# fwrnke/pseudo-3D-interpolation

Measured on AMD Instinct MI355X. Metric: POCS iterations/s on the 1024x1024x512 cube, higher is better.
Workload: dtype complex64 (f32 arithmetic)

## Files before the change

### pseudo-3d-interpolation_amd/csrc/p3d_api.hip

```cpp
#include <hip/hip_runtime.h>

#include <climits>
#include <cmath>
#include <algorithm>
#include <cstdlib>
#include <cstring>
#include <string>
#include <thread>
#include <vector>

#include "p3d.h"
#include "p3d_generic.hpp"
#include "p3d_host.hpp"
#include "p3d_internal.hpp"
#include "p3d_flex.hpp"
#include "p3d_mix_entry.hpp"
#include "p3d_resident.hpp"
#include "p3d_select.hpp"
#include "p3d_kernels.hpp"

namespace p3d {
#define P3D_DECL(n) const LineOps* get_line_ops_##n();
P3D_DECL(2) P3D_DECL(4) P3D_DECL(8) P3D_DECL(16) P3D_DECL(32) P3D_DECL(64) P3D_DECL(128) P3D_DECL(256)
P3D_DECL(512) P3D_DECL(1024) P3D_DECL(2048) P3D_DECL(4096)
// ... 226 lines not shown
{
    const int wpl = tpl >= 64 ? tpl / 64 : 1, rpw = tpl >= 64 ? 1 : 64 / tpl;
    const int unit = blockIdx.x * blockDim.x + threadIdx.x;
    if (unit >= n1 / rpw) return;
    unsigned run = rowbase[unit * rpw];
    for (int j = 0; j < 16 * wpl; ++j) {
        const size_t w = (size_t)unit * wpl * 16 + j;
        cbase[w] = run;
        run += (unsigned)__popcll(bits64[w]);
    }
}

static __global__ void pack_mask32_kernel(const uint16_t* bits, unsigned long long* bits32, int n1)
{
    const int i = blockIdx.x * blockDim.x + threadIdx.x;
    if (i >= (n1 / 2) * 32) return;
    const int k = i & 31, u = i >> 5;
    unsigned long long w = 0;
    for (int l = 0; l < 64; ++l) {
        const int row = 2 * u + (l >> 5), c = (l & 31) + 32 * k;
        w |= (unsigned long long)((bits[(size_t)row * 64 + (c & 63)] >> (c >> 6)) & 1u) << l;
    }
    bits32[i] = w;
}

static thread_local std::string g_err;

namespace p3d { void set_last_error(const char* msg) { g_err = msg; } }

struct p3d_plan {
    int device = 0;
    int nil = 0, nxl = 0, max_slices = 0;
    hipStream_t stream = nullptr;
    p3d_plan* pct_plan = nullptr;
    unsigned* pct_sel = nullptr;
    unsigned* pct_hist = nullptr;
    float* pct_frac = nullptr;
    bool generic = false;
    GenPlan gcol{}, grow{};
    static constexpr int GEN_STAT_BLOCKS = 64;
    const LineOps* ops_col = nullptr;
    const LineOps* ops_row = nullptr;
    c32 *tw_col = nullptr, *tw_row = nullptr;
    c32* work = nullptr;
    uint8_t* nzflag = nullptr;
    uint16_t* nzm = nullptr;
    unsigned long long* nzcount = nullptr;
    bool sparse_ok = false;
    double last_nonzero_fraction = -1.0;
    uint16_t* bits = nullptr;
    unsigned long long* bits64 = nullptr;
    unsigned long long* nzl = nullptr;
    unsigned* cbase = nullptr;
    unsigned long long* mbits = nullptr;
    unsigned* mbase = nullptr;
    const p3d::mix::Entry* mix_row = nullptr;
    bool mix_binary = false;
    bool use32 = false;
    unsigned long long* bits32 = nullptr;
    c32* tw32 = nullptr;
    int* flag = nullptr;
    unsigned* rowbase = nullptr;
    char* xc = nullptr;
    size_t xc_cap = 0;
    double* sums = nullptr;
    size_t sums_cap = 0;
    double* rowsum = nullptr;
    c32* tau = nullptr;
    size_t tau_cap = 0;
    int* done = nullptr;
    float* partials = nullptr;
    int tiles = 0;
    int cus = 0;
    int pipe_wgs = 0;
    int host_sw = 0;
    int flex_over = 0;
    bool no_colpipe = false;
    void* st_x = nullptr;
    void* st_out = nullptr;
    float* st_mask = nullptr;
    size_t st_cap = 0;
    struct Primed { bool valid = false; const void* x = nullptr; const float* mask = nullptr; int dtype = 0, nslices = 0, nonbinary = 0, violation = 0; unsigned nobs = 0;
                    bool real = false;
    } primed;
    double* sum0 = nullptr;
    int sorted_slices = 0;
    hipEvent_t ev0 = nullptr, ev1 = nullptr;
    std::vector<hipEvent_t> prof_events;
    double prof_col_ms = 0, prof_row_ms = 0;
    int prof_col_n = 0, prof_row_n = 0;

    size_t slice_elems() const { return (size_t)nil * nxl; }
};

static int upload_table(p3d_plan* p, const LineOps* ops, bool for_rows, int n, c32** dst)
{
    std::vector<c32> host;
    if (is_flex(ops)) {
        flex_build_table(n, host);
    } else {
        host.resize(for_rows ? (size_t)ops->row_tw_slots : (size_t)ops->col_tw_slots);
        if (for_rows) ops->build_row_tw(host.data());
        else ops->build_col_tw(host.data());
    }
    P3D_TRY(hipMalloc((void**)dst, sizeof(c32) * host.size()));
    P3D_TRY(hipMemcpy(*dst, host.data(), sizeof(c32) * host.size(), hipMemcpyHostToDevice));
    return P3D_OK;
}

extern "C" {

int p3d_abi_version(void) { return P3D_ABI_VERSION; }

const char* p3d_last_error(void) { return g_err.c_str(); }

int p3d_runtime_info(int* compiled_hip_version, int* runtime_hip_version)
{
    if (!compiled_hip_version || !runtime_hip_version) return fail(P3D_ERR_INVALID, "NULL argument");
    *compiled_hip_version = HIP_VERSION;
    P3D_TRY(hipRuntimeGetVersion(runtime_hip_version));
    return P3D_OK;
}

int p3d_device_count(int* n)
{
    if (!n) return fail(P3D_ERR_INVALID, "n is NULL");
    *n = 0;
    P3D_TRY(hipGetDeviceCount(n));
    return P3D_OK;
}

static bool generic_ok(int n) { return n >= 1 && n <= GEN_MAX_N && gen_make_plan(n).nf >= 0; }

int p3d_shape_supported(int nil, int nxl)
{
    if (find_ops(nil) != nullptr && find_ops(nxl) != nullptr) return 1;
    return (generic_ok(nil) && generic_ok(nxl)) ? 1 : 0;
}

int p3d_plan_destroy(p3d_plan* p)
{
    if (!p) return P3D_OK;
    if (p->pct_plan) p3d_plan_destroy(p->pct_plan);
    hipSetDevice(p->device);
    if (p->stream) hipStreamSynchronize(p->stream);
    void* bufs[] = {p->mbits, p->mbase, p->cbase, p->bits64, p->bits32, p->tw32, p->nzl, p->nzflag, p->nzm, p->nzcount, p->tw_col, p->tw_row, p->work, p->bits, p->flag, p->rowbase, p->xc, p->sums, p->rowsum, p->sum0, p->tau, p->pct_sel, p->pct_hist, p->pct_frac,
                    p->done,   p->partials, p->st_x, p->st_out, p->st_mask};
    for (void* b : bufs)
        if (b) hipFree(b);
    for (hipEvent_t e : p->prof_events) hipEventDestroy(e);
    if (p->ev0) hipEventDestroy(p->ev0);
    if (p->ev1) hipEventDestroy(p->ev1);
    if (p->stream) hipStreamDestroy(p->stream);
    delete p;
    return P3D_OK;
}

static int create_plan(p3d_plan** out, int device, int nil, int nxl, int max_slices, bool force_generic)
{
    if (!out) return fail(P3D_ERR_INVALID, "out is NULL");
    *out = nullptr;
    if (nil < 1 || nxl < 1 || max_slices < 1) return fail(P3D_ERR_INVALID, "nil, nxl and max_slices must be positive");
    if (max_slices > 65535) return fail(P3D_ERR_INVALID, "max_slices > 65535: split the cube into batches");
    const LineOps* oc = find_ops(nil);
    const LineOps* orow = find_ops(nxl);
    const bool generic = !oc || !orow || force_generic;
// ... 142 lines not shown
    if (!dst || !src) return fail(P3D_ERR_INVALID, "NULL argument");
    P3D_TRY(hipSetDevice(device));
    P3D_TRY(hipMemcpy(dst, src, bytes, kind == 0 ? hipMemcpyHostToDevice : kind == 1 ? hipMemcpyDeviceToHost : hipMemcpyDeviceToDevice));
    if (kind == 2) P3D_TRY(hipDeviceSynchronize());
    return P3D_OK;
}

int p3d_dev_memset(int device, void* dptr, int value, size_t bytes)
{
    if (!bytes) return P3D_OK;
    if (!dptr) return fail(P3D_ERR_INVALID, "NULL argument");
    P3D_TRY(hipSetDevice(device));
    P3D_TRY(hipMemset(dptr, value, bytes));
    P3D_TRY(hipDeviceSynchronize());
    return P3D_OK;
}

int p3d_dev_synchronize(int device)
{
    P3D_TRY(hipSetDevice(device));
    P3D_TRY(hipDeviceSynchronize());
    return P3D_OK;
}

int p3d_dev_mem_info(int device, size_t* free_bytes, size_t* total_bytes)
{
    if (!free_bytes || !total_bytes) return fail(P3D_ERR_INVALID, "NULL argument");
    if (int rc = use_device(device)) return rc;
    P3D_TRY(hipMemGetInfo(free_bytes, total_bytes));
    return P3D_OK;
}

int p3d_host_alloc(void** hptr, size_t bytes)
{
    if (!hptr) return fail(P3D_ERR_INVALID, "NULL argument");
    P3D_TRY(hipHostMalloc(hptr, bytes, hipHostMallocDefault));
    return P3D_OK;
}

int p3d_host_free(void* hptr)
{
    P3D_TRY(hipHostFree(hptr));
    return P3D_OK;
}

int p3d_memcpy_h2d(p3d_plan* p, void* dst, const void* src, size_t bytes)
{
    if (!p) return fail(P3D_ERR_INVALID, "NULL plan");
    P3D_TRY(hipSetDevice(p->device));
    P3D_TRY(hipMemcpyAsync(dst, src, bytes, hipMemcpyHostToDevice, p->stream));
    P3D_TRY(hipStreamSynchronize(p->stream));
    return P3D_OK;
}

int p3d_memcpy_d2h(p3d_plan* p, void* dst, const void* src, size_t bytes)
{
    if (!p) return fail(P3D_ERR_INVALID, "NULL plan");
    P3D_TRY(hipSetDevice(p->device));
    P3D_TRY(hipMemcpyAsync(dst, src, bytes, hipMemcpyDeviceToHost, p->stream));
    P3D_TRY(hipStreamSynchronize(p->stream));
    return P3D_OK;
}

int p3d_host_register(void* hptr, size_t bytes)
{
    if (!hptr || bytes == 0) return fail(P3D_ERR_INVALID, "NULL argument");
    const hipError_t e = hipHostRegister(hptr, bytes, hipHostRegisterDefault);
    if (e != hipSuccess) {
        (void)hipGetLastError();
        return fail(P3D_ERR_UNSUPPORTED, "hipHostRegister refused %zu bytes at %p: %s", bytes, hptr, hipGetErrorString(e));
    }
    return P3D_OK;
}

int p3d_host_unregister(void* hptr)
{
    if (!hptr) return fail(P3D_ERR_INVALID, "NULL argument");
    P3D_TRY(hipHostUnregister(hptr));
    return P3D_OK;
}

}

struct RunSwitches { bool no_pct_fused; bool no_mask_bits, no_compact, no_real, no_sparse, real_2048, no_resident, no_tstore, force_colpipe, no_colpipe; };
static RunSwitches read_switches()
{
    RunSwitches s;
    s.no_pct_fused = getenv("P3D_NO_PCT_FUSED") != nullptr;
    s.no_mask_bits = getenv("P3D_NO_MASK_BITS") != nullptr;
    s.no_compact = getenv("P3D_NO_COMPACT") != nullptr;
    s.no_real = getenv("P3D_NO_REAL") != nullptr;
    s.no_sparse = getenv("P3D_NO_SPARSE") != nullptr;
    s.real_2048 = getenv("P3D_NO_REAL_2048") == nullptr;
    s.no_resident = getenv("P3D_NO_RESIDENT") != nullptr;
    s.no_tstore = getenv("P3D_NO_TSTORE") != nullptr;
    s.force_colpipe = getenv("P3D_FORCE_COLPIPE") != nullptr;
    s.no_colpipe = getenv("P3D_NO_COLPIPE") != nullptr;
    return s;
}

static int check_batch(p3d_plan* p, int nslices)
{
    if (!p) return fail(P3D_ERR_INVALID, "NULL plan");
    p->primed.valid = false;
    p->sorted_slices = 0;
    if (nslices < 1 || nslices > p->max_slices)
        return fail(P3D_ERR_INVALID, "nslices = %d outside 1..max_slices (%d)", nslices, p->max_slices);
    return P3D_OK;
}

static RowArgs row_args(p3d_plan* p, int nslices)
{
    RowArgs r{};
    r.tw = p->tw_row;
    r.tw32 = p->tw32;
    r.n1 = p->nil;
    r.nslices = nslices;
    r.alpha = 1.0f;
    r.scale = (float)(1.0 / ((double)p->nil * (double)p->nxl));
    r.len = p->nxl;
    r.host_sw = p->host_sw;
    return r;
}

static ColArgs col_args(p3d_plan* p, int nslices)
{
    ColArgs c{};
    c.tw = p->tw_col;
    c.n2 = p->nxl;
    c.nslices = nslices;
    c.len = p->nil;
    c.cus = p->cus;
    c.host_sw = p->host_sw;
    c.flex_over = p->flex_over;
    return c;
}

static int ensure_staging(p3d_plan* p, size_t bytes_per_cube)
{
    if (p->st_cap >= bytes_per_cube && p->st_x) return P3D_OK;
    if (p->st_x) hipFree(p->st_x);
    if (p->st_out) hipFree(p->st_out);
    p->st_x = p->st_out = nullptr;
    p->st_cap = 0;
    P3D_TRY(hipMalloc(&p->st_x, bytes_per_cube));
    P3D_TRY(hipMalloc(&p->st_out, bytes_per_cube));
    if (!p->st_mask) P3D_TRY(hipMalloc((void**)&p->st_mask, sizeof(float) * p->slice_elems()));
    p->st_cap = bytes_per_cube;
    return P3D_OK;
}


static int gen_fft2(p3d_plan* p, const c32* in, c32* out, int nslices, int inverse, const int* done)
{
    const float scale = (float)(1.0 / ((double)p->nil * (double)p->nxl));
    if (!inverse) {
        P3D_TRY(gen_launch_line_fft(in, out, p->tw_row, p->grow, FWD, 1.0f, nslices, p->nil, p->nxl, true, done, p->stream));
        P3D_TRY(gen_launch_line_fft(out, out, p->tw_col, p->gcol, FWD, 1.0f, nslices, p->nil, p->nxl, false, done, p->stream));
    } else {
        P3D_TRY(gen_launch_line_fft(in, out, p->tw_col, p->gcol, INV, 1.0f, nslices, p->nil, p->nxl, false, done, p->stream));
        P3D_TRY(gen_launch_line_fft(out, out, p->tw_row, p->grow, INV, scale, nslices, p->nil, p->nxl, true, done, p->stream));
    }
    return P3D_OK;
}

static int reduce_partials(p3d_plan* p, int nslices, double* stats, int tiles = 0)
{
    if (tiles <= 0) tiles = p->tiles;
    std::vector<float> part((size_t)STATS_PARTIAL * tiles * nslices);
    P3D_TRY(hipMemcpyAsync(part.data(), p->partials, sizeof(float) * part.size(), hipMemcpyDeviceToHost, p->stream));
    P3D_TRY(hipStreamSynchronize(p->stream));
    for (int s = 0; s < nslices; ++s) {
        double lr = -INFINITY, li = -INFINITY, mx = 0.0, mn = INFINITY, sq = 0.0;
        for (int t = 0; t < tiles; ++t) {
            const float* q = &part[((size_t)s * tiles + t) * STATS_PARTIAL];
            if (q[0] > lr || (q[0] == lr && q[1] > li)) { lr = q[0]; li = q[1]; }
            if (q[2] > mx) mx = q[2];
            if (q[3] < mn) mn = q[3];
            sq += q[4];
        }
// ... 287 lines not shown
    if (p->use32) pack_mask32_kernel<<<((p->nil / 2) * 32 + 255) / 256, 256, 0, p->stream>>>(p->bits, p->bits32, p->nil);
    P3D_TRY(hipGetLastError());
    P3D_TRY(hipMemcpyAsync(nonbinary, p->flag, sizeof(int), hipMemcpyDeviceToHost, p->stream));
    if (p->nil <= 4096) P3D_TRY(hipMemcpyAsync(nobs, p->rowbase + p->nil, sizeof(unsigned), hipMemcpyDeviceToHost, p->stream));
    P3D_TRY(hipStreamSynchronize(p->stream));
    return P3D_OK;
}

static bool want_compact(p3d_plan* p, int nonbinary, unsigned nobs, int niter, const RunSwitches& sw)
{
    return !nonbinary && p->pipe_wgs > 0 && p->nil <= 4096 && niter > 1 && !sw.no_compact && nobs > 0 &&
           (double)nobs < 0.75 * (double)p->slice_elems();
}

static int ensure_xc(p3d_plan* p, int nslices, unsigned nobs, int dtype)
{
    return grow(p->xc, p->xc_cap, (size_t)nslices * nobs * (dtype == P3D_C64 ? sizeof(c32) : sizeof(float)));
}

int p3d_pocs_prime_dev(p3d_plan* p, const void* x, int dtype, const float* mask, int nslices, double* stats)
{
    int rc = check_batch(p, nslices);
    if (rc) return rc;
    if (!x || !mask || !stats) return fail(P3D_ERR_INVALID, "NULL buffer");
    if (dtype != P3D_C64 && dtype != P3D_F32) return fail(P3D_ERR_INVALID, "unknown dtype %d", dtype);
    P3D_TRY(hipSetDevice(p->device));
    if (p->generic || is_flex(p->ops_row) || is_flex(p->ops_col)) return p3d_pocs_stats_dev(p, x, dtype, nslices, stats);
    const RunSwitches sw = read_switches();
    int nonbinary = 0;
    unsigned nobs = 0;
    if ((rc = pack_mask(p, mask, &nonbinary, &nobs))) return rc;
    if (sw.no_mask_bits) nonbinary = 1;
    const bool compact = want_compact(p, nonbinary, nobs, 2, sw);
    if (compact && (rc = ensure_xc(p, nslices, nobs, dtype))) return rc;
    RowArgs r = row_args(p, nslices);
    r.x = x;
    r.mask = nonbinary ? mask : nullptr;
    r.bits = nonbinary ? nullptr : p->bits;
    r.bits64 = nonbinary ? nullptr : p->bits64;
    r.cbase = nonbinary ? nullptr : p->cbase;
    r.bits32 = (nonbinary || !p->use32) ? nullptr : p->bits32;
    r.xc = compact ? p->xc : nullptr;
    r.rowbase = p->rowbase;
    r.nobs = nobs;
    r.violation = p->flag + 1;
    r.work = p->work;
    r.sums = p->rowsum;
    r.dtype = dtype;
    r.real_2048 = sw.real_2048 ? 1 : 0;
    P3D_TRY(hipMemsetAsync(p->rowsum, 0, sizeof(double) * (size_t)p->nil * nslices, p->stream));
    bool real = dtype == P3D_F32 && !sw.no_real && compact && r.bits64 && r.cbase && p->pipe_wgs > 0 && p->ops_row->row_real != nullptr;
    if (real) {
        const hipError_t re = p->ops_row->row_real(REAL_FIRST, r, p->pipe_wgs, p->stream);
        if (re == hipErrorNotSupported) real = false;
        else P3D_TRY(re);
    }
    int violation = 0;
    if (real) {
        P3D_TRY(hipMemcpyAsync(&violation, p->flag + 1, sizeof(int), hipMemcpyDeviceToHost, p->stream));
        P3D_TRY(hipStreamSynchronize(p->stream));
        if (violation) {
            real = false;
            P3D_TRY(hipMemsetAsync(p->rowsum, 0, sizeof(double) * (size_t)p->nil * nslices, p->stream));
        }
    }
    if (!real) P3D_TRY(first_row_pass(p, r));
    reduce_rows_kernel<<<nslices, 256, 0, p->stream>>>(p->rowsum, p->sum0, p->nil);
    ColArgs c = col_args(p, nslices);
    c.in = p->work;
    c.partials = p->partials;
    int tiles = p->tiles;
    if (real) {
        c.n2 = p->nxl / 2 + 1;
        c.herm_n2 = p->nxl;
        tiles = (c.n2 + p->ops_col->col_tile - 1) / p->ops_col->col_tile;
    }
    P3D_TRY(p->ops_col->col(COL_STATS, c, p->stream));
    if (compact && !real) P3D_TRY(hipMemcpyAsync(&violation, p->flag + 1, sizeof(int), hipMemcpyDeviceToHost, p->stream));
    if ((rc = reduce_partials(p, nslices, stats, tiles))) return rc;
    p->primed.valid = true;
    p->primed.x = x; p->primed.mask = mask; p->primed.dtype = dtype; p->primed.nslices = nslices;
    p->primed.nonbinary = nonbinary; p->primed.nobs = nobs; p->primed.violation = violation;
    p->primed.real = real;
    return P3D_OK;
}

int p3d_pocs_stats_dev(p3d_plan* p, const void* x, int dtype, int nslices, double* stats)
{
    int rc = check_batch(p, nslices);
    if (rc) return rc;
    if (!x || !stats) return fail(P3D_ERR_INVALID, "NULL buffer");
    if (dtype != P3D_C64 && dtype != P3D_F32) return fail(P3D_ERR_INVALID, "unknown dtype %d", dtype);
    P3D_TRY(hipSetDevice(p->device));
    if (p->generic) {
        P3D_TRY(hipMemsetAsync(p->rowsum, 0, sizeof(double) * nslices, p->stream));
        P3D_TRY(gen_launch_update(p->work, x, dtype, nullptr, nullptr, p->rowsum, 0, 0, 0, 1.0f, nslices, p->slice_elems(), nullptr, 0,
                                  p->stream));
        if ((rc = gen_fft2(p, p->work, p->work, nslices, 0, nullptr))) return rc;
        P3D_TRY(gen_launch_stats(p->work, p->partials, nslices, p->slice_elems(), p->tiles, p->stream));
        return reduce_partials(p, nslices, stats);
    }
    RowArgs r = row_args(p, nslices);
    r.x = x;
    r.work = p->work;
    r.dtype = dtype;
    P3D_TRY(first_row_pass(p, r));
    ColArgs c = col_args(p, nslices);
    c.in = p->work;
    c.partials = p->partials;
    P3D_TRY(p->ops_col->col(COL_STATS, c, p->stream));
    return reduce_partials(p, nslices, stats);
}

int p3d_pocs_stats(p3d_plan* p, const void* x, int dtype, int nslices, double* stats)
{
    int rc = check_batch(p, nslices);
    if (rc) return rc;
    if (!x || !stats) return fail(P3D_ERR_INVALID, "NULL buffer");
    if (dtype != P3D_C64 && dtype != P3D_F32) return fail(P3D_ERR_INVALID, "unknown dtype %d", dtype);
    P3D_TRY(hipSetDevice(p->device));
    if ((rc = ensure_staging(p, sizeof(c32) * p->slice_elems() * p->max_slices))) return rc;
    const size_t esz = dtype == P3D_C64 ? sizeof(c32) : sizeof(float);
    P3D_TRY(hipMemcpy(p->st_x, x, esz * p->slice_elems() * nslices, hipMemcpyHostToDevice));
    return p3d_pocs_stats_dev(p, p->st_x, dtype, nslices, stats);
}

struct RunJob {
    p3d_plan* p;
    const void* x;
    int dtype;
    const float* mask;
    const double* tau;
    const p3d_pocs_params* prm;
    void* out;
    int nslices;
    int32_t* niter_done;
    double* sums;
    double* elapsed_ms;
    int base_op;
    bool percentile;
    RunSwitches sw;
    LoopFrame frame;
};

static int run_generic(RunJob& j)
{
    p3d_plan* const p = j.p;
    const p3d_pocs_params* const prm = j.prm;
    const void* const x = j.x;
    const float* const mask = j.mask;
    const double* const tau = j.tau;
    void* const out = j.out;
    const int dtype = j.dtype, nslices = j.nslices, niter = prm->niter, base_op = j.base_op;
    const bool percentile = j.percentile, early = prm->eps > 0.0, adaptive = prm->version == P3D_VER_ADAPTIVE;
    int rc;
    const size_t per_slice = p->slice_elems();
    const int* done_d = (early || j.frame.any_off()) ? p->done : nullptr;
    P3D_TRY(gen_launch_update(p->work, x, dtype, mask, out, p->sums, 0, adaptive ? 1 : 0, 0, (float)prm->alpha, nslices, per_slice,
                              done_d, 0, p->stream));
    for (int k = 0; k < niter; ++k) {
        const bool last = k + 1 == niter;
        if ((rc = gen_fft2(p, p->work, p->work, nslices, 0, done_d))) return rc;
        if (percentile) {
            std::vector<unsigned> sel_h((size_t)nslices * 16, 0u);
            std::vector<float> frac_h(nslices);
            for (int s = 0; s < nslices; ++s)
// ... 74 lines not shown
    r.bits64 = nonbinary ? nullptr : p->bits64;
    r.cbase = nonbinary ? nullptr : p->cbase;
    r.bits32 = (nonbinary || !p->use32) ? nullptr : p->bits32;
    r.xc = compact ? p->xc : nullptr;
    r.rowbase = p->rowbase;
    r.nobs = nobs;
    r.violation = p->flag + 1;
    r.work = p->work;
    r.out = out;
    const bool any_off = early || j.frame.any_off();
    r.sums = p->rowsum;
    r.done = any_off ? p->done : nullptr;
    r.dtype = dtype;
    r.real_2048 = sw.real_2048 ? 1 : 0;
    r.tstore = sw.no_tstore ? 0 : 1;
    r.adaptive = adaptive ? 1 : 0;
    const bool finalize = early && !adaptive;
    r.write_out = (early && !finalize) ? 1 : 0;
    r.alpha = (float)prm->alpha;
    r.sum_row = 0;
    P3D_TRY(hipMemsetAsync(p->rowsum, 0, sizeof(double) * (size_t)p->nil * nslices, p->stream));
    bool real_path = dtype == P3D_F32 && base_op == P3D_OP_HARD && !adaptive && !percentile && p->ops_row->row_real != nullptr && !sw.no_real &&
                     (flex_rows ? p->nil % 2 == 0 : (compact && r.bits64 && r.cbase && p->pipe_wgs > 0));
    const bool primed_real = primed_in && primed_state.real && real_path;
    if (real_path && !primed_real) {
        const hipError_t re = p->ops_row->row_real(REAL_FIRST, r, p->pipe_wgs, p->stream);
        if (re == hipErrorNotSupported) real_path = false;
        else P3D_TRY(re);
    }
    bool mix_compact = false;
    if (flex_rows && p->mix_binary && !real_path && !sw.no_mask_bits) {
        r.mbits = p->mbits;
        r.mbase = p->mbase;
        mix_compact = niter > 1 && !sw.no_compact && nobs > 0 && (double)nobs < 0.75 * (double)p->slice_elems();
        if (mix_compact) {
            if ((rc = ensure_xc(p, nslices, nobs, dtype))) return rc;
            r.xc = p->xc;
        }
    }
    const bool primed = primed_in && !adaptive && (real_path ? primed_real : !primed_state.real);
    if (primed) {
        P3D_TRY(hipMemcpyAsync(p->sums, p->sum0, sizeof(double) * nslices, hipMemcpyDeviceToDevice, p->stream));
        if (any_off) zero_off_sums_kernel<<<(nslices + 255) / 256, 256, 0, p->stream>>>(p->sums, p->done, nslices);
        if (primed_state.violation) r.xc = nullptr;
    } else if (!real_path) {
        P3D_TRY(first_row_pass(p, r));
    }
    if ((compact || mix_compact) && !primed) {
        int violation = 0;
        P3D_TRY(hipMemcpyAsync(&violation, p->flag + 1, sizeof(int), hipMemcpyDeviceToHost, p->stream));
        P3D_TRY(hipStreamSynchronize(p->stream));
        if (violation) {
            r.xc = nullptr;
            if (real_path) {
                real_path = false;
                P3D_TRY(hipMemsetAsync(p->rowsum, 0, sizeof(double) * (size_t)p->nil * nslices, p->stream));
                P3D_TRY(first_row_pass(p, r));
            }
        }
    }
    if (!primed) reduce_rows_kernel<<<nslices, 256, 0, p->stream>>>(p->rowsum, p->sums, p->nil);

    ColArgs c = col_args(p, nslices);
    c.in = p->work;
    c.out = p->work;
    c.tau = p->tau;
    c.done = any_off ? p->done : nullptr;
    c.niter = niter;
    c.op = base_op;
    const bool sparse = p->sparse_ok && !sw.no_sparse && !percentile;
    const int nblocks = (p->nxl + 7) / 8, groups = flex_rows ? 1 : p->ops_row->tpl / 8;
    const int col_t = is_flex(p->ops_col) ? flex_col_tile(p->nil) : p->ops_col->col_tile;
    if (sparse) {
        c.nzflag = p->nzflag;
        r.zero_off = (unsigned)(wk_slice_stride(p->nil, p->nxl) * (size_t)p->max_slices);
        P3D_TRY(hipMemsetAsync(p->nzcount, 0, sizeof(unsigned long long), p->stream));
    }
    const bool colpipe = sparse && p->cus > 0 && p->ops_col->col_pipe != nullptr &&
                         (sw.force_colpipe || (p->ops_col->n >= 2048 && !sw.no_colpipe));
    p->last_nonzero_fraction = -1.0;
    const int n2_work = real_path ? p->nxl / 2 + 1 : p->nxl;
    const int tiles_work = (n2_work + col_t - 1) / col_t;
    c.n2 = n2_work;

    std::vector<unsigned> pct_sel_h;
    std::vector<float> pct_frac_h;
    if (percentile) {
        const size_t per_slice = p->slice_elems();
        if (!p->pct_sel) {
            P3D_TRY(hipMalloc((void**)&p->pct_sel, sizeof(unsigned) * 16 * (size_t)p->max_slices));
            P3D_TRY(hipMalloc((void**)&p->pct_hist, sizeof(unsigned) * 2048 * (size_t)p->max_slices));
            P3D_TRY(hipMalloc((void**)&p->pct_frac, sizeof(float) * (size_t)p->max_slices));
        }
        pct_sel_h.assign((size_t)niter * nslices * 16, 0u);
        pct_frac_h.assign((size_t)niter * nslices, 0.f);
        for (int k = 0; k < niter; ++k)
            for (int s = 0; s < nslices; ++s) {
                unsigned* sel = &pct_sel_h[(size_t)k * nslices * 16];
                percentile_rank(tau[2 * ((size_t)s * niter + k)], per_slice, &sel[(size_t)s * 8], &sel[((size_t)nslices + s) * 8], &pct_frac_h[(size_t)k * nslices + s]);
            }
        P3D_TRY(hipMemsetAsync(p->pct_hist, 0, sizeof(unsigned) * 2048 * (size_t)nslices, p->stream));
    }

    const bool no_sums = !early && sums == nullptr;
    const bool fam32 = !real_path && p->use32 && r.xc != nullptr && r.bits32 != nullptr;
    if (no_sums && fam32 && !adaptive) r.sums = nullptr;
    P3D_TRY(stamp());
    int last_finalized = 0;
    const bool check_done_rows = finalize && getenv("P3D_CHECK_DONE_ROWS") != nullptr;
    std::vector<unsigned long long> done_sum_first(check_done_rows ? nslices : 0, 0ull), done_sum_now(check_done_rows ? nslices : 0, 0ull);
    std::vector<char> done_sum_seen(check_done_rows ? nslices : 0, 0);
    unsigned long long* done_sum_d = nullptr;
    if (check_done_rows) P3D_TRY(hipMalloc((void**)&done_sum_d, sizeof(unsigned long long) * nslices));
    struct FreeSum { unsigned long long* p; ~FreeSum() { if (p) hipFree(p); } } free_sum{done_sum_d};
    for (int k = 0; k < niter; ++k) {
        c.iter = k;
        if (percentile) {
            const size_t per_slice = p->slice_elems();
            ColArgs cf = c;
            cf.tau = nullptr;
            cf.nzflag = nullptr;
            P3D_TRY(p->ops_col->col(COL_FWD, cf, p->stream));
            P3D_TRY(hipMemcpyAsync(p->pct_sel, &pct_sel_h[(size_t)k * nslices * 16], sizeof(unsigned) * 16 * (size_t)nslices, hipMemcpyHostToDevice, p->stream));
            P3D_TRY(hipMemcpyAsync(p->pct_frac, &pct_frac_h[(size_t)k * nslices], sizeof(float) * nslices, hipMemcpyHostToDevice, p->stream));
            for (int which = 0; which < 2; ++which) {
                unsigned* sel = p->pct_sel + (size_t)which * nslices * 8;
                for (int level = 0; level < 3; ++level) {
                    P3D_TRY(gen_launch_pct_hist(p->work, per_slice, sel, p->pct_hist, level, nslices, p->stream));
                    P3D_TRY(gen_launch_pct_scan(sel, p->pct_hist, level, nslices, p->stream));
                }
            }
            P3D_TRY(gen_launch_pct_tau(p->pct_sel, p->pct_sel + (size_t)nslices * 8, p->pct_frac, p->tau, niter, k, nslices, p->stream));
            P3D_TRY(gen_launch_shrink(p->work, p->tau, niter, k, base_op, nslices, per_slice, c.done, p->stream));
            P3D_TRY(p->ops_col->col(COL_INV, cf, p->stream));
        } else {
            hipError_t ce = hipErrorNotSupported;
            if (colpipe) ce = p->ops_col->col_pipe(c, p->cus, p->stream);
            if (ce == hipErrorNotSupported) ce = p->ops_col->col(COL_ITER, c, p->stream);
            P3D_TRY(ce);
        }
        if (sparse && real_path && !flex_rows) {
            nz_real_kernel<<<(nslices * 16 * (p->ops_row->tpl >= 64 ? p->ops_row->tpl / 64 : 1) + 3) / 4, 256, 0, p->stream>>>(p->nzflag, p->nzl, p->nzcount, nslices, tiles_work, col_t, p->nxl, p->ops_row->tpl, c.done);
            r.nzl = p->nzl;
        } else if (sparse && flex_rows) {
            const int nb_work = (n2_work + 7) / 8;
            nz_count_kernel<<<(nslices * nb_work + 255) / 256, 256, 0, p->stream>>>(p->nzflag, p->nzcount, nslices, tiles_work, col_t, nb_work, c.done);
            r.nzflag = p->nzflag;
            r.nz_tiles = tiles_work;
            r.nz_col_t = col_t;
        } else if (sparse) {
            nz_pack_kernel<<<(nslices * groups + 255) / 256, 256, 0, p->stream>>>(p->nzflag, p->nzm, p->nzcount, nslices, p->tiles, col_t, groups, nblocks,
                                                                                c.done, p->nzl);
            r.nzm = p->nzm;
            r.nzl = p->nzl;
        }
        P3D_TRY(stamp());
        r.sum_row = k + 1;
        bool piped = false;
        if (real_path) {
            P3D_TRY(p->ops_row->row_real(k + 1 < niter ? REAL_MID : REAL_LAST, r, p->pipe_wgs, p->stream));
            piped = true;
        } else if (fam32) {
            const hipError_t fe = p->ops_row->row_pipe32(k + 1 < niter ? PIPE_MID : PIPE_LAST, r, p->pipe_wgs, p->stream);
            if (fe == hipErrorNotSupported) return fail(P3D_ERR_HIP, "row_pipe32_kernel refused a job its first pass had accepted");
            P3D_TRY(fe);
            piped = true;
        } else if (k + 1 < niter && p->pipe_wgs > 0) {
            const hipError_t pe = p->ops_row->row_pipe(r, p->pipe_wgs, p->stream);
            if (pe == hipSuccess) piped = true;
            else if (pe != hipErrorNotSupported) P3D_TRY(pe);
        }
        if (!piped && k + 1 == niter && p->pipe_wgs > 0 && p->bits64 != nullptr && p->ops_row->row_pipe64 != nullptr) {
            const hipError_t le = p->ops_row->row_pipe64(PIPE_LAST, r, p->pipe_wgs, p->stream);
            if (le == hipSuccess) piped = true;
            else if (le != hipErrorNotSupported) P3D_TRY(le);
        }
        if (!piped) P3D_TRY(p->ops_row->row(k + 1 < niter ? ROW_MID : ROW_LAST, r, p->stream));
        P3D_TRY(stamp());
        if (!no_sums) reduce_rows_kernel<<<nslices, 256, 0, p->stream>>>(p->rowsum, p->sums + (size_t)(k + 1) * nslices, p->nil);
        if (early) {
            conv_kernel<<<(nslices + 255) / 256, 256, 0, p->stream>>>(p->sums, p->done, nslices, k, prm->eps);
            P3D_TRY(hipMemsetAsync(p->rowsum, 0, sizeof(double) * (size_t)p->nil * nslices, p->stream));
            constexpr int FIN_EVERY = 8;
            if (check_done_rows) {
                done_rows_checksum_kernel<<<nslices, 256, 0, p->stream>>>(reinterpret_cast<const unsigned long long*>(p->work), wk_slice_stride(p->nil, n2_work),
                                                                         p->done, last_finalized, done_sum_d);
                P3D_TRY(hipMemcpyAsync(done_sum_now.data(), done_sum_d, sizeof(unsigned long long) * nslices, hipMemcpyDeviceToHost, p->stream));
                P3D_TRY(hipMemcpyAsync(done_h.data(), p->done, sizeof(int) * nslices, hipMemcpyDeviceToHost, p->stream));
                P3D_TRY(hipStreamSynchronize(p->stream));
                for (int s = 0; s < nslices; ++s) {
                    if (done_h[s] <= last_finalized) continue;
                    if (!done_sum_seen[s]) { done_sum_seen[s] = 1; done_sum_first[s] = done_sum_now[s]; }
                    else if (done_sum_first[s] != done_sum_now[s])
                        return fail(P3D_ERR_HIP, "P3D_CHECK_DONE_ROWS: the work rows of slice %d (converged at iteration %d) changed before its finalize launch (iteration %d)", s,
                                    done_h[s], k + 1);
                }
            }
            if (finalize && k + 1 < niter && (k + 1 - last_finalized >= FIN_EVERY || k + 2 >= niter)) {
                RowArgs f = r;
                f.nzm = nullptr;
                f.nzl = nullptr;
                f.nzflag = nullptr;
                f.only_done_lo = last_finalized;
                f.only_done = k + 1;
                last_finalized = k + 1;
                f.plain = 0;
                f.sums = nullptr;
                f.done = p->done;
                f.scale = (float)(1.0 / (double)p->nxl);
                if (real_path) P3D_TRY(p->ops_row->row_real(REAL_LAST, f, p->pipe_wgs, p->stream));
                else P3D_TRY(p->ops_row->row(ROW_LAST, f, p->stream));
            }
        }
    }
    P3D_TRY(hipGetLastError());
    if ((rc = j.frame.enqueue_end(sums))) return rc;
    unsigned long long kept_blocks = 0;
    if (sparse) P3D_TRY(hipMemcpyAsync(&kept_blocks, p->nzcount, sizeof kept_blocks, hipMemcpyDeviceToHost, p->stream));
    if ((rc = j.frame.collect(j.niter_done, j.elapsed_ms))) return rc;
    if (sparse) p->last_nonzero_fraction = (double)kept_blocks / ((double)niter * nslices * (real_path ? (n2_work + 7) / 8 : nblocks));
// ... 355 lines not shown
```

### pseudo-3d-interpolation_amd/csrc/p3d_col_kernels.hpp

```cpp
#pragma once

#include "p3d_kernels_common.hpp"

namespace p3d {

__device__ __forceinline__ bool lex_greater(float ar, float ai, float br, float bi)
{
    return (ar > br) || (ar == br && ai > bi);
}

template <int N, int T, int MODE>
__global__ __launch_bounds__(T* Plan<N>::TPL, (T * Plan<N>::TPL >= 1024 ? 4 : P3D_WAVES_PER_EU)) void col_kernel(const ColArgs a)
{
    using PL = Plan<N>;
    constexpr int TPL = PL::TPL, PPT = PL::PPT;
    constexpr int THREADS = T * TPL;
    constexpr int CW = T < 8 ? T : 8;
    using LDS = LdsColW<CW>;
    extern __shared__ __attribute__((aligned(16))) unsigned char smem_raw[];
    c32* twl = reinterpret_cast<c32*>(smem_raw);
    c32* data = twl + ColTables<N>::slots();
    const TwCol tw{twl};

    const int tid = threadIdx.x;
    const int c_lo = tid % CW;
    const int tl = (tid / CW) % TPL;
    const int cbl = tid / (CW * TPL);
    const int slice = blockIdx.y;
    int tile = blockIdx.x;
    if constexpr (T < 8) {
        constexpr int G = 8 / T;
        if (P3D_XCD_PAIR && (gridDim.x % (8 * G)) == 0) {
            const int xcd = tile & 7, j = tile >> 3;
            tile = ((j / G) * 8 + xcd) * G + (j % G);
        }
    }
    const int col = tile * T + cbl * CW + c_lo;
    const bool valid = col < a.n2;

    if (a.done && a.done[slice] != 0) return;

    for (int i = tid; i < ColTables<N>::slots(); i += THREADS) twl[i] = a.tw[i];
    __syncthreads();

    const LDS lds{data + cbl * LDS::stride(N) + c_lo};
    constexpr bool ITER = MODE == COL_ITER || MODE == COL_ITER_SOFT || MODE == COL_ITER_GARROTE;
    const int vcol = valid ? col : 0;
    const c32* const inb = a.in + (size_t)slice * (a.in_std ? (size_t)N * a.n2 : wk_slice_stride(N, a.n2));
    c32* const outb = a.out + (size_t)slice * (a.out_std ? (size_t)N * a.n2 : wk_slice_stride(N, a.n2));
    const unsigned blk0 = ((unsigned)(vcol >> 3) * N) * 8 + (vcol & 7);
    const bool in_std = !ITER && a.in_std, out_std = !ITER && a.out_std;
    const unsigned in_org = in_std ? (unsigned)vcol : blk0, in_pitch = in_std ? (unsigned)a.n2 : 8u;
    const unsigned out_org = out_std ? (unsigned)vcol : blk0, out_pitch = out_std ? (unsigned)a.n2 : 8u;
    auto eoff = [&](int std_layout, int r) -> unsigned {
        return std_layout ? (unsigned)r * a.n2 + vcol : blk0 + (unsigned)r * 8;
    };
    c32 v[PPT];
    if (MODE == COL_SHRINK) {
        const int b = slice / a.sh.nsh, s = slice - b * a.sh.nsh;
        const c32 tau = a.sh.tau[((size_t)b * a.sh.niter + a.sh.iter) * a.sh.nsh + s];
        const float scale = 1.0f / ((float)N * (float)a.n2);
        unsigned rows_on = 0;
#pragma unroll
        for (int q = 0; q < PPT; ++q) rows_on |= (shear_group_on(a.sh, s, (tl + TPL * q) >> 3) ? 1u : 0u) << q;
#pragma unroll
        for (int q = 0; q < PPT; ++q) v[q] = ((rows_on >> q) & 1u) ? inb[eoff(0, tl + TPL * q)] : c32{0.f, 0.f};
        line_fft<N, INV, false>(v, lds, tw, tl);
        const Shrink shr(tau, a.sh.op);
#pragma unroll
        for (int q = 0; q < PPT; ++q) {
            c32 c = v[q] * scale;
            if (a.sh.real_only) c.y = 0.f;
            v[q] = shr(c);
        }
        line_fft<N, FWD, false>(v, lds, tw, tl);
        if (valid) {
#pragma unroll
            for (int q = 0; q < PPT; ++q)
                if ((rows_on >> q) & 1u) outb[eoff(0, tl + TPL * q)] = v[q];
        }
        return;
    }
#pragma unroll
    for (int q = 0; q < PPT; ++q)
        v[q] = *reinterpret_cast<const c32*>(reinterpret_cast<const char*>(inb) + (in_org + (unsigned)(tl + TPL * q) * in_pitch) * 8u);

    if (MODE != COL_INV) line_fft<N, FWD, false>(v, lds, tw, tl);

    if (ITER || (MODE == COL_FWD && a.tau != nullptr)) {
        const c32 tau = a.tau[(size_t)slice * a.niter + a.iter];
        const int op = MODE == COL_ITER ? 0 : (MODE == COL_ITER_SOFT ? 1 : (MODE == COL_ITER_GARROTE ? 2 : a.op));
        const Shrink shr(tau, op);
#pragma unroll
        for (int q = 0; q < PPT; ++q) v[q] = shr(v[q]);
        if (ITER && a.nzflag != nullptr) {
            unsigned bits = 0;
#pragma unroll
            for (int q = 0; q < PPT; ++q) bits |= __float_as_uint(v[q].x) | __float_as_uint(v[q].y);
            const int kept = __syncthreads_or(bits != 0u ? 1 : 0);
            if (tid == 0) a.nzflag[(size_t)slice * gridDim.x + tile] = kept ? 1 : 0;
            if (!kept) {
                if constexpr (T < 8) {
                    if (valid) {
#pragma unroll
                        for (int q = 0; q < PPT; ++q) {
                            unsigned o = (out_org + (unsigned)(tl + TPL * q) * out_pitch) * 8u;
                            asm volatile("" : "+v"(o));
                            *reinterpret_cast<c32*>(reinterpret_cast<char*>(outb) + o) = c32{0.f, 0.f};
                        }
                    }
                }
                return;
            }
        }
    }

    if (MODE == COL_STATS) {
        float lr = -INFINITY, li = -INFINITY, mx = 0.f, mn = INFINITY, sq = 0.f;
        if (valid) {
            const bool twice = a.herm_n2 > 0 && col != 0 && 2 * col != a.herm_n2;
#pragma unroll
            for (int q = 0; q < PPT; ++q) {
                const float p = v[q].x * v[q].x + v[q].y * v[q].y;
                const float vi = twice ? fabsf(v[q].y) : v[q].y;
                if (lex_greater(v[q].x, vi, lr, li)) { lr = v[q].x; li = vi; }
                mx = fmaxf(mx, p);
                mn = fminf(mn, p);
                sq += p;
            }
            if (twice) sq += sq;
        }
        const int lane = tid & 63;
        const int nact = (THREADS - (tid & ~63)) < 64 ? (THREADS - (tid & ~63)) : 64;
#pragma unroll
        for (int o = 32; o > 0; o >>= 1) {
            const float orr = __shfl_down(lr, o, 64), oi = __shfl_down(li, o, 64);
            const float omx = __shfl_down(mx, o, 64), omn = __shfl_down(mn, o, 64), osq = __shfl_down(sq, o, 64);
            if (lane + o < nact) {
                if (lex_greater(orr, oi, lr, li)) { lr = orr; li = oi; }
                mx = fmaxf(mx, omx);
                mn = fminf(mn, omn);
                sq += osq;
            }
        }
        __syncthreads();
        float* red = reinterpret_cast<float*>(data);
        const int wave = tid >> 6, nw = (THREADS + 63) >> 6;
        if ((tid & 63) == 0) {
            red[wave * 5 + 0] = lr; red[wave * 5 + 1] = li; red[wave * 5 + 2] = mx;
            red[wave * 5 + 3] = mn; red[wave * 5 + 4] = sq;
        }
        __syncthreads();
        if (tid == 0) {
            for (int w = 1; w < nw; ++w) {
                if (lex_greater(red[w * 5], red[w * 5 + 1], lr, li)) { lr = red[w * 5]; li = red[w * 5 + 1]; }
                mx = fmaxf(mx, red[w * 5 + 2]);
                mn = fminf(mn, red[w * 5 + 3]);
                sq += red[w * 5 + 4];
            }
            float* p = a.partials + ((size_t)slice * gridDim.x + blockIdx.x) * STATS_PARTIAL;
            p[0] = lr; p[1] = li; p[2] = sqrtf(mx); p[3] = sqrtf(mn); p[4] = sq;
        }
        return;
    }

    if (ITER || MODE == COL_INV) line_fft<N, INV, false>(v, lds, tw, tl);

    if (valid) {
#pragma unroll
        for (int q = 0; q < PPT; ++q) {
            unsigned o = (out_org + (unsigned)(tl + TPL * q) * out_pitch) * 8u;
            asm volatile("" : "+v"(o));
            *reinterpret_cast<c32*>(reinterpret_cast<char*>(outb) + o) = v[q];
        }
    }
}

#ifndef P3D_COLPIPE_WAVES_PER_EU
#define P3D_COLPIPE_WAVES_PER_EU 4
#endif
template <int N, int T, int OP, bool SHEAR = false>
__global__ __launch_bounds__(T* Plan<N>::TPL, P3D_COLPIPE_WAVES_PER_EU) void col_pipe_kernel(const ColArgs a)
{
    using PL = Plan<N>;
    constexpr int TPL = PL::TPL, PPT = PL::PPT;
    constexpr int THREADS = T * TPL;
    static_assert(T % 8 == 0 && PPT == 16, "whole 64-byte column blocks per tile");
    constexpr int CW = 8;
    using LDS = LdsColW<CW>;
    extern __shared__ __attribute__((aligned(16))) unsigned char smem_raw[];
    c32* twl = reinterpret_cast<c32*>(smem_raw);
    c32* data = twl + ColTables<N>::slots();
    const TwCol tw{twl};

    const int tid = threadIdx.x;
    const int c_lo = tid % CW;
    const int tl = (tid / CW) % TPL;
    const int cbl = tid / (CW * TPL);
    for (int i = tid; i < ColTables<N>::slots(); i += THREADS) twl[i] = a.tw[i];
    __syncthreads();
    const LDS lds{data + cbl * LDS::stride(N) + c_lo};

    const unsigned tiles = (unsigned)(a.n2 + T - 1) / T;
    const unsigned total = (unsigned)a.nslices * tiles;
    const size_t sstride = wk_slice_stride(N, a.n2);
    const unsigned slice_bytes = (unsigned)(sstride * 8);
    typedef const int __attribute__((address_space(4))) * kint_t;
    const kint_t k_done = (kint_t)a.done;
    typedef const unsigned long long __attribute__((address_space(4))) * ktau_t;
    const ktau_t k_tau = (ktau_t)(SHEAR ? a.sh.tau : a.tau);
    struct Tile { unsigned slice, tile; bool on; };
    auto locate = [&](unsigned g) -> Tile {
        Tile t;
        t.on = g < total;
        const unsigned gg = t.on ? g : 0u;
        t.slice = gg / tiles;
        t.tile = gg - t.slice * tiles;
        if (k_done != nullptr && t.on && k_done[t.slice] != 0) t.on = false;
        return t;
    };
    auto lane_off = [&](const Tile& t, bool& valid) -> unsigned {
        const int col = (int)t.tile * T + cbl * CW + c_lo;
        valid = col < a.n2;
        const int vcol = valid ? col : 0;
        return (((unsigned)(vcol >> 3) * N) * 8 + (vcol & 7) + (unsigned)tl * 8) * 8u;
    };
    typedef const unsigned __attribute__((address_space(4))) * ksup_t;
    const ksup_t k_sup = (ksup_t)a.sh.sup;
    auto rows_of = [&](const Tile& t) -> unsigned {
        if constexpr (!SHEAR) return 0xffffu;
        if (k_sup == nullptr) return 0xffffu;
        const unsigned sh = t.slice % (unsigned)a.sh.nsh;
        const unsigned g0 = (unsigned)__builtin_amdgcn_readfirstlane(tl >> 3);
        unsigned m = 0;
#pragma unroll
        for (int q = 0; q < PPT; ++q) {
            const unsigned g = g0 + (unsigned)(TPL / 8) * q;
            m |= ((k_sup[(size_t)sh * a.sh.sup_words + (g >> 5)] >> (g & 31u)) & 1u) << q;
        }
        return m;
    };
    auto issue = [&](raw64 (&dst)[PPT], const Tile& t) {
        bool valid;
        const unsigned vo = lane_off(t, valid);
// ... 79 lines not shown
```

### pseudo-3d-interpolation_amd/csrc/p3d_kernels_common.hpp

```cpp
#pragma once

#include <hip/hip_runtime.h>
#include <stdint.h>

#include "p3d_fft.hpp"
#include "p3d_shrink.hpp"

#ifndef P3D_ROW_THREADS
#define P3D_ROW_THREADS 256
#endif
#ifndef P3D_WAVES_PER_EU
#define P3D_WAVES_PER_EU 4
#endif
#ifndef P3D_XO_GROUP
#define P3D_XO_GROUP 4
#endif
#ifndef P3D_XO_EARLY
#define P3D_XO_EARLY 0
#endif
#ifndef P3D_XCD_PAIR
#define P3D_XCD_PAIR 1
#endif
#ifndef P3D_PIPE_WAVES_PER_EU
#define P3D_PIPE_WAVES_PER_EU 2
#endif
#ifndef P3D_PIPE_WAVES_PER_EU_COMPACT
#define P3D_PIPE_WAVES_PER_EU_COMPACT 3
#endif
#ifndef P3D_COMPACT_LATE
#define P3D_COMPACT_LATE 1
#endif
#ifndef P3D_PIPE_LOCKSTEP
#define P3D_PIPE_LOCKSTEP 1
#endif
#ifndef P3D_PIPE_PREFETCH
#define P3D_PIPE_PREFETCH 1
#endif
#ifndef P3D_ROW_WAVES_PER_EU
#define P3D_ROW_WAVES_PER_EU (P3D_ROW_THREADS >= 512 ? 4 : 3)
#endif

namespace p3d {

enum RowMode { ROW_FIRST = 0, ROW_MID = 1, ROW_LAST = 2, ROW_SPREAD_INV = 3, ROW_GATHER_FWD = 4 };
enum ColMode { COL_ITER = 0, COL_STATS = 1, COL_FWD = 2, COL_INV = 3, COL_ITER_SOFT = 4, COL_ITER_GARROTE = 5,
               COL_SHRINK = 6 };

struct ShearArgs {
    const float* psi;
    const c32* tau;
    int nsh, niter, iter, op, real_only;
    const unsigned* sup;
    int sup_words;
    int half;
};
__host__ __device__ inline int shear_rows(const ShearArgs& sh, int n1) { return sh.half ? n1 / 2 + 1 : n1; }
__device__ __forceinline__ bool shear_group_on(const ShearArgs& sh, int s, int g)
{
    return sh.sup == nullptr || ((sh.sup[(size_t)s * sh.sup_words + (g >> 5)] >> (g & 31)) & 1u) != 0u;
}

#ifndef P3D_ROW1024_MAXMODE
#define P3D_ROW1024_MAXMODE 2
#endif
constexpr int ROW_THREADS = P3D_ROW_THREADS;
template <int N, int MODE>
constexpr int row_threads() { return (N == 1024 && MODE <= P3D_ROW1024_MAXMODE && P3D_ROW_THREADS < 1024) ? 1024 : P3D_ROW_THREADS; }
constexpr int STATS_PARTIAL = 8;

__host__ __device__ inline size_t wk_slice_stride(int n1, int n2) { return (size_t)((n2 + 7) / 8) * 8 * n1; }
__host__ __device__ inline size_t wk_off(int row, int col, int n1) { return ((size_t)(col >> 3) * n1 + row) * 8 + (col & 7); }


template <int TPL>
__device__ __forceinline__ unsigned wk_lane_off(int tl, int row, unsigned wblk)
{
    if constexpr (TPL % 8 == 0) return (unsigned)(tl >> 3) * wblk + (unsigned)row * 8 + (tl & 7);
    else return (unsigned)row * 8;
}
template <int TPL, class P>
__device__ __forceinline__ P wk_q_ptr(P ws, int q, int tl, unsigned wblk)
{
    if constexpr (TPL % 8 == 0) return ws + (size_t)q * (TPL / 8) * wblk;
    else { const int e = tl + TPL * q; return ws + (size_t)(e >> 3) * wblk + (e & 7); }
}

template <int TPL>
struct CompactIndex {
    unsigned long long line_mask;
    unsigned long long below;
    unsigned running;
    __device__ __forceinline__ CompactIndex(int lane, unsigned base)
    {
        const int first = lane & ~(TPL - 1);
        line_mask = TPL == 64 ? ~0ull : (((1ull << TPL) - 1ull) << first);
        below = line_mask & ((1ull << lane) - 1ull);
        running = base;
    }
    __device__ __forceinline__ unsigned next(bool set)
    {
        const unsigned long long b = __ballot(set);
        const unsigned idx = running + (unsigned)__popcll(b & below);
        running += (unsigned)__popcll(b & line_mask);
        return idx;
    }
};

__host__ __device__ constexpr size_t pipe64_word(size_t row_or_slice, int wpl, int wsub, int q) { return (row_or_slice * wpl + wsub) * 16 + q; }

enum { P3D_SW_FLEX_NO_PERSIST = 1, P3D_SW_FLEX_NO_INPLACE = 2 };

struct RowArgs {
    const void* x;
    const float* mask;
    const uint16_t* bits;
    void* xc;
    const unsigned* rowbase;
    unsigned nobs;
    int* violation;
    c32* work;
    void* out;
    const c32* tw;
    double* sums;
    const int* done;
    int n1;
    int nslices;
    int sum_row;
    int dtype;
    int adaptive;
    int write_out;
    int plain;
    const uint16_t* nzm;
    unsigned zero_off;
    const uint8_t* nzflag;
    int nz_tiles;
    int nz_col_t;
    int only_done_lo;
    int only_done;
    const unsigned long long* bits64;
    const unsigned long long* nzl;
    const unsigned* cbase;
    const unsigned long long* bits32;
    const c32* tw32;
    const unsigned long long* mbits;
    const unsigned* mbase;
    float alpha;
    float scale;
    int len;
    int real_2048;
    int tstore;
    int host_sw;
    ShearArgs sh;
};

struct ColArgs {
    const c32* in;
    c32* out;
    const c32* tw;
    const c32* tau;
    const int* done;
    float* partials;
    int n2;
    int nslices;
    int niter;
    int iter;
    int op;
    int in_std;
    int out_std;
    ShearArgs sh;
    int len;
    uint8_t* nzflag;
    int cus;
    int host_sw;
    int flex_over;
    int herm_n2;
};

__device__ __forceinline__ float abs_c32(c32 v) { return __builtin_amdgcn_sqrtf(v.x * v.x + v.y * v.y); }

__device__ __forceinline__ double wave_sum(double v)
{
#pragma unroll
    for (int o = 32; o > 0; o >>= 1) v += __shfl_down(v, o, 64);
    return v;
}

typedef unsigned p3d_u2 __attribute__((ext_vector_type(2)));
constexpr unsigned BUF_OOB = 0x80000000u;
__device__ __forceinline__ __amdgpu_buffer_rsrc_t buf_srd(const void* base, unsigned bytes)
{
    return __builtin_amdgcn_make_buffer_rsrc(const_cast<void*>(base), 0, (int)bytes, 0x00020000);
}
typedef unsigned long long raw64;
__device__ __forceinline__ raw64 buf_load_raw64(__amdgpu_buffer_rsrc_t r, unsigned voff, unsigned soff)
{
    const p3d_u2 t = __builtin_amdgcn_raw_buffer_load_b64(r, (int)voff, (int)soff, 0);
    return (raw64)t.x | ((raw64)t.y << 32);
}
__device__ __forceinline__ c32 raw_c32(raw64 u) { return c32{__uint_as_float((unsigned)u), __uint_as_float((unsigned)(u >> 32))}; }
__device__ __forceinline__ c32 buf_load_c32(__amdgpu_buffer_rsrc_t r, unsigned voff, unsigned soff) { return raw_c32(buf_load_raw64(r, voff, soff)); }
__device__ __forceinline__ float buf_load_f32(__amdgpu_buffer_rsrc_t r, unsigned voff, unsigned soff)
{
    return __uint_as_float(__builtin_amdgcn_raw_buffer_load_b32(r, (int)voff, (int)soff, 0));
}
__device__ __forceinline__ void buf_store_c32(__amdgpu_buffer_rsrc_t r, unsigned voff, unsigned soff, c32 v)
{
    __builtin_amdgcn_raw_buffer_store_b64(p3d_u2{__float_as_uint(v.x), __float_as_uint(v.y)}, r, (int)voff, (int)soff, 0);
}
typedef unsigned p3d_u4 __attribute__((ext_vector_type(4)));
__device__ __forceinline__ void buf_store_2c32(__amdgpu_buffer_rsrc_t r, unsigned voff, unsigned soff, c32 a, c32 b)
{
    __builtin_amdgcn_raw_buffer_store_b128(p3d_u4{__float_as_uint(a.x), __float_as_uint(a.y), __float_as_uint(b.x), __float_as_uint(b.y)}, r,
                                           (int)voff, (int)soff, 0);
}
__device__ __forceinline__ void buf_store_f64(__amdgpu_buffer_rsrc_t r, unsigned voff, unsigned soff, double v)
{
    const unsigned long long u = (unsigned long long)__double_as_longlong(v);
    __builtin_amdgcn_raw_buffer_store_b64(p3d_u2{(unsigned)u, (unsigned)(u >> 32)}, r, (int)voff, (int)soff, 0);
}

}
```

Before: 429.1.

## Skip first-iteration column tiles whose stats peak is below threshold

The stats pass now records a per-tile squared-magnitude peak in the partials buffer. On the first hard-threshold iteration, the column iteration kernel reads that peak and, when it falls below the shrink limit, marks the tile as all-zero in the sparsity flag and exits before the FFT. To use this, the first iteration bypasses the column pipeline path. The goal is to avoid FFT and threshold work on tiles that would be zeroed anyway, at the cost of losing colpipe for that iteration and depending on the stats partials staying valid between priming and the run.

```diff
diff --git a/pseudo-3d-interpolation_amd/csrc/p3d_api.hip b/pseudo-3d-interpolation_amd/csrc/p3d_api.hip
--- a/pseudo-3d-interpolation_amd/csrc/p3d_api.hip
+++ b/pseudo-3d-interpolation_amd/csrc/p3d_api.hip
@@ -332,6 +332,7 @@
     size_t st_cap = 0;
     struct Primed { bool valid = false; const void* x = nullptr; const float* mask = nullptr; int dtype = 0, nslices = 0, nonbinary = 0, violation = 0; unsigned nobs = 0;
                     bool real = false;
+                    bool tile_peaks = false;
     } primed;
     double* sum0 = nullptr;
     int sorted_slices = 0;
@@ -640,7 +641,7 @@
 
 }
 
-struct RunSwitches { bool no_pct_fused; bool no_mask_bits, no_compact, no_real, no_sparse, real_2048, no_resident, no_tstore, force_colpipe, no_colpipe; };
+struct RunSwitches { bool no_pct_fused; bool no_mask_bits, no_compact, no_real, no_sparse, real_2048, no_resident, no_tstore, force_colpipe, no_colpipe, no_tile_peaks; };
 static RunSwitches read_switches()
 {
     RunSwitches s;
@@ -654,6 +655,7 @@
     s.no_tstore = getenv("P3D_NO_TSTORE") != nullptr;
     s.force_colpipe = getenv("P3D_FORCE_COLPIPE") != nullptr;
     s.no_colpipe = getenv("P3D_NO_COLPIPE") != nullptr;
+    s.no_tile_peaks = getenv("P3D_NO_TILE_PEAKS") != nullptr;
     return s;
 }
 
@@ -1107,6 +1109,7 @@
     p->primed.x = x; p->primed.mask = mask; p->primed.dtype = dtype; p->primed.nslices = nslices;
     p->primed.nonbinary = nonbinary; p->primed.nobs = nobs; p->primed.violation = violation;
     p->primed.real = real;
+    p->primed.tile_peaks = true;
     return P3D_OK;
 }
 
@@ -1347,6 +1350,7 @@
     const int n2_work = real_path ? p->nxl / 2 + 1 : p->nxl;
     const int tiles_work = (n2_work + col_t - 1) / col_t;
     c.n2 = n2_work;
+    const bool tile_peaks = primed && primed_state.tile_peaks && sparse && base_op == P3D_OP_HARD && !sw.no_tile_peaks && !sw.force_colpipe;
 
     std::vector<unsigned> pct_sel_h;
     std::vector<float> pct_frac_h;
@@ -1400,7 +1404,8 @@
             P3D_TRY(p->ops_col->col(COL_INV, cf, p->stream));
         } else {
             hipError_t ce = hipErrorNotSupported;
-            if (colpipe) ce = p->ops_col->col_pipe(c, p->cus, p->stream);
+            c.tile_mx = (tile_peaks && k == 0) ? p->partials + STATS_TILE_MX : nullptr;
+            if (colpipe && c.tile_mx == nullptr) ce = p->ops_col->col_pipe(c, p->cus, p->stream);
             if (ce == hipErrorNotSupported) ce = p->ops_col->col(COL_ITER, c, p->stream);
             P3D_TRY(ce);
         }
diff --git a/pseudo-3d-interpolation_amd/csrc/p3d_col_kernels.hpp b/pseudo-3d-interpolation_amd/csrc/p3d_col_kernels.hpp
--- a/pseudo-3d-interpolation_amd/csrc/p3d_col_kernels.hpp
+++ b/pseudo-3d-interpolation_amd/csrc/p3d_col_kernels.hpp
@@ -40,11 +40,34 @@
 
     if (a.done && a.done[slice] != 0) return;
 
+    constexpr bool ITER = MODE == COL_ITER || MODE == COL_ITER_SOFT || MODE == COL_ITER_GARROTE;
+    typedef const unsigned long long __attribute__((address_space(4))) * ktau_t;
+    unsigned long long tau_bits = 0;
+    if constexpr (ITER) tau_bits = ((ktau_t)a.tau)[(size_t)slice * a.niter + a.iter];
+
+    if constexpr (MODE == COL_ITER) {
+        if (a.tile_mx != nullptr && a.nzflag != nullptr && (tile + 1) * T <= a.n2) {
+            typedef const float __attribute__((address_space(4))) * kmx_t;
+            const float mx = ((kmx_t)a.tile_mx)[((size_t)slice * gridDim.x + blockIdx.x) * STATS_PARTIAL];
+            const Shrink shr(c32{__uint_as_float((unsigned)tau_bits), __uint_as_float((unsigned)(tau_bits >> 32))}, 0);
+            if (mx < shr.lim) {
+                if (tid == 0) a.nzflag[(size_t)slice * gridDim.x + tile] = 0;
+                if constexpr (T < 8) {
+                    if (valid) {
+                        c32* const ob = a.out + (size_t)slice * wk_slice_stride(N, a.n2) + (((unsigned)(col >> 3) * N) * 8 + (col & 7));
+#pragma unroll
+                        for (int q = 0; q < PPT; ++q) ob[(unsigned)(tl + TPL * q) * 8] = c32{0.f, 0.f};
+                    }
+                }
+                return;
+            }
+        }
+    }
+
     for (int i = tid; i < ColTables<N>::slots(); i += THREADS) twl[i] = a.tw[i];
     __syncthreads();
 
     const LDS lds{data + cbl * LDS::stride(N) + c_lo};
-    constexpr bool ITER = MODE == COL_ITER || MODE == COL_ITER_SOFT || MODE == COL_ITER_GARROTE;
     const int vcol = valid ? col : 0;
     const c32* const inb = a.in + (size_t)slice * (a.in_std ? (size_t)N * a.n2 : wk_slice_stride(N, a.n2));
     c32* const outb = a.out + (size_t)slice * (a.out_std ? (size_t)N * a.n2 : wk_slice_stride(N, a.n2));
@@ -88,7 +111,7 @@
     if (MODE != COL_INV) line_fft<N, FWD, false>(v, lds, tw, tl);
 
     if (ITER || (MODE == COL_FWD && a.tau != nullptr)) {
-        const c32 tau = a.tau[(size_t)slice * a.niter + a.iter];
+        const c32 tau = ITER ? c32{__uint_as_float((unsigned)tau_bits), __uint_as_float((unsigned)(tau_bits >> 32))} : a.tau[(size_t)slice * a.niter + a.iter];
         const int op = MODE == COL_ITER ? 0 : (MODE == COL_ITER_SOFT ? 1 : (MODE == COL_ITER_GARROTE ? 2 : a.op));
         const Shrink shr(tau, op);
 #pragma unroll
@@ -160,6 +183,7 @@
             }
             float* p = a.partials + ((size_t)slice * gridDim.x + blockIdx.x) * STATS_PARTIAL;
             p[0] = lr; p[1] = li; p[2] = sqrtf(mx); p[3] = sqrtf(mn); p[4] = sq;
+            p[STATS_TILE_MX] = sq != sq ? INFINITY : mx;
         }
         return;
     }
diff --git a/pseudo-3d-interpolation_amd/csrc/p3d_kernels_common.hpp b/pseudo-3d-interpolation_amd/csrc/p3d_kernels_common.hpp
--- a/pseudo-3d-interpolation_amd/csrc/p3d_kernels_common.hpp
+++ b/pseudo-3d-interpolation_amd/csrc/p3d_kernels_common.hpp
@@ -67,6 +67,7 @@
 template <int N, int MODE>
 constexpr int row_threads() { return (N == 1024 && MODE <= P3D_ROW1024_MAXMODE && P3D_ROW_THREADS < 1024) ? 1024 : P3D_ROW_THREADS; }
 constexpr int STATS_PARTIAL = 8;
+constexpr int STATS_TILE_MX = 5;
 
 __host__ __device__ inline size_t wk_slice_stride(int n1, int n2) { return (size_t)((n2 + 7) / 8) * 8 * n1; }
 __host__ __device__ inline size_t wk_off(int row, int col, int n1) { return ((size_t)(col >> 3) * n1 + row) * 8 + (col & 7); }
@@ -174,6 +175,7 @@
     int host_sw;
     int flex_over;
     int herm_n2;
+    const float* tile_mx;
 };
 
 __device__ __forceinline__ float abs_c32(c32 v) { return __builtin_amdgcn_sqrtf(v.x * v.x + v.y * v.y); }
```

Result: no change. 428.5 (-0.1%).
